# Stansfash/nonstationary-precip

Hardware: AMD Instinct MI355X
Metric: dsvi_elbo_steps_per_sec (higher is better)
Workload: dtype f32; 1 GPU; 2-layer DSVI DeepGP (hidden 3->2 + last 2->1), M=1024, S=10, minibatch 4096 (global, split over the GPUs) of synthetic N=1e5 spatio-temporal grid; fwd+ELBO+bwd+Adam; M=1024, S=10, per_gpu_batch=4096, global_batch=4096, N=100000, parallelism=dp1, kzz_cholesky_dtype=f64, hipgraph=True

## Files before the change

nonstationary-precip_amd/csrc/gemm.hip:

```cpp
#include <cstdlib>
#include <type_traits>
#include "common.h"

namespace {

constexpr int F64_BK = 16;
constexpr int F64_DEPTH = 2;
constexpr int F64ACC_BN = 64;
constexpr int F64ACC_BK = 16;

#ifdef NSGP_GEMM_STAMPS
__device__ unsigned long long* nsgp_stamp_buf = nullptr;
__device__ unsigned long long nsgp_stamp_cap = 0;
#define NSGP_STAMP(i) do { if (threadIdx.x == 0) stamp_v[i] = __builtin_amdgcn_s_memtime(); } while (0)
#define NSGP_STAMP_FLUSH() do { \
        if (threadIdx.x == 0 && nsgp_stamp_buf) { \
            const unsigned long long si = (unsigned long long)blockIdx.y * gridDim.x + blockIdx.x; \
            if (si < nsgp_stamp_cap) { \
                unsigned long long* sp = nsgp_stamp_buf + si * 16; \
                sp[0] = stamp_v[0]; sp[1] = stamp_v[1]; sp[2] = stamp_v[2]; sp[3] = __builtin_amdgcn_s_memtime(); \
                sp[4] = stamp_rt0; sp[5] = __builtin_amdgcn_s_memrealtime(); \
                sp[6] = ((unsigned long long)(unsigned)bm << 40) | ((unsigned long long)(unsigned)bn << 16) | (unsigned)nt; \
                sp[8] = stamp_bar; \
                sp[7] = ((unsigned long long)__builtin_amdgcn_s_getreg(63508) << 32) | (unsigned)__builtin_amdgcn_s_getreg(63492); \
            } \
        } } while (0)
#define NSGP_LOOP_BARRIER() do { \
        const unsigned long long b0_ = __builtin_amdgcn_s_memtime(); \
        __syncthreads(); \
        stamp_bar += __builtin_amdgcn_s_memtime() - b0_; \
    } while (0)
#else
#define NSGP_STAMP(i) do { } while (0)
#define NSGP_STAMP_FLUSH() do { } while (0)
#define NSGP_LOOP_BARRIER() __syncthreads()
#endif

template <typename T> struct Mfma;
template <> struct Mfma<float> {
    static constexpr int MT = 32, KS = 2, NREG = 16, PAD = 4;
    typedef float acc_t __attribute__((ext_vector_type(16)));
    static __device__ __forceinline__ acc_t mma(float a, float b, acc_t c) {
        return __builtin_amdgcn_mfma_f32_32x32x2f32(a, b, c, 0, 0, 0);
    }
    static __device__ __forceinline__ int krow(int lane) { return lane >> 5; }
    static __device__ __forceinline__ int mcol(int lane) { return lane & 31; }
    static __device__ __forceinline__ int crow(int r, int lane) { return (r & 3) + 8 * (r >> 2) + 4 * (lane >> 5); }
    static __device__ __forceinline__ int crow_lane(int lane) { return 4 * (lane >> 5); }
    static __device__ __forceinline__ constexpr int crow_reg(int r) { return (r & 3) + 8 * (r >> 2); }
    static __device__ __forceinline__ int ccol(int lane) { return lane & 31; }
};
template <> struct Mfma<double> {
    static constexpr int MT = 16, KS = 4, NREG = 4, PAD = 16;
    typedef double acc_t __attribute__((ext_vector_type(4)));
    static __device__ __forceinline__ acc_t mma(double a, double b, acc_t c) {
        return __builtin_amdgcn_mfma_f64_16x16x4f64(a, b, c, 0, 0, 0);
    }
    static __device__ __forceinline__ int krow(int lane) { return lane >> 4; }
    static __device__ __forceinline__ int mcol(int lane) { return lane & 15; }
    static __device__ __forceinline__ int crow(int r, int lane) { return (lane >> 4) + 4 * r; }
    static __device__ __forceinline__ int crow_lane(int lane) { return lane >> 4; }
    static __device__ __forceinline__ constexpr int crow_reg(int r) { return 4 * r; }
    static __device__ __forceinline__ int ccol(int lane) { return lane & 15; }
};

struct GemmArgs {
    int64_t M, N, K;
    int64_t sam, sak, sa1, sa2;
    int64_t sbk, sbn, sb1, sb2;
    int64_t ldc, sc1, sc2;
    int64_t nb2;
    int64_t tiles_m, tiles_n;
    int64_t ksplit, kper;
    int64_t slab;
    int flags;
    int nbk;
    int part_rows;
    int xcd_chunk;
    int xcd_group;
    int batch_perm;
    int vecA, vecB;
    int modeA, modeB;
};

struct Epi {
    int kind;
    const void *rv, *cs, *gc, *mat, *ks;
    void *p0, *p1;
    int modeA, modeB;
    int part_rows;
    int p64;
    const float *kz, *kx, *kls, *kos;
    int kD;
    int64_t kx_sx;
};
constexpr int KGEN_DMAX = 4;

template <typename T> struct Frag4 { T v[4]; };

template <typename T> __device__ __forceinline__ Frag4<T> ldg4(const T* p) {
    Frag4<T> f;
    if constexpr (sizeof(T) == 4) {
        const float4 q = *reinterpret_cast<const float4*>(p);
        f.v[0] = q.x; f.v[1] = q.y; f.v[2] = q.z; f.v[3] = q.w;
    } else {
        const double2 q0 = *reinterpret_cast<const double2*>(p);
        const double2 q1 = *reinterpret_cast<const double2*>(p + 2);
        f.v[0] = q0.x; f.v[1] = q0.y; f.v[2] = q1.x; f.v[3] = q1.y;
    }
    return f;
}

template <typename T, int MODE, int BR, int BK, int P>
struct TileLoader {
    static constexpr int TPK = BK / 4, TPR = BR / 4;
    static constexpr int RS = MODE == 0 ? 256 / TPK : 0;
    static constexpr int KS = MODE == 0 ? 0 : 256 / TPR;
    int r0, k0;
    const T* cur;
    int64_t pstep, kstep;
    __device__ __forceinline__ void init(int tid, const T* base, int64_t row0, int64_t sr, int64_t sk, int64_t kbeg) {
        if (MODE == 0) { r0 = tid / TPK; k0 = (tid % TPK) * 4; }
        else { r0 = (tid % TPR) * 4; k0 = tid / TPR; }
        kstep = sk;
        pstep = MODE == 0 ? RS * sr : KS * sk;
        cur = base + (row0 + r0) * sr + (kbeg + k0) * sk;
    }
    __device__ __forceinline__ int prow(int p) const { return r0 + p * RS; }
    __device__ __forceinline__ int pk(int p) const { return k0 + p * KS; }
    __device__ __forceinline__ void load_fast(Frag4<T>* f, int64_t koff) const {
#pragma unroll
        for (int p = 0; p < P; ++p) f[p] = ldg4(cur + p * pstep + koff * kstep);
    }
    __device__ __forceinline__ void load_edge(Frag4<T>* f, const T* base, int64_t row0, int64_t sr, int64_t sk, int64_t k0g,
                                              int rrem, int krem) const {
#pragma unroll
        for (int p = 0; p < P; ++p)
#pragma unroll
            for (int e = 0; e < 4; ++e) {
                const int r = prow(p) + (MODE == 0 ? 0 : e), k = pk(p) + (MODE == 0 ? e : 0);
                f[p].v[e] = (r < rrem && k < krem) ? base[(row0 + r) * sr + (k0g + k) * sk] : T(0);
            }
    }
    __device__ __forceinline__ void mask_piece(Frag4<T>& f, int p, int d, bool zgt, bool zlt) const {
#pragma unroll
        for (int e = 0; e < 4; ++e) {
            const int r = prow(p) + (MODE == 0 ? 0 : e), k = pk(p) + (MODE == 0 ? e : 0) + d;
            const bool z = (zgt && k > r) || (zlt && k < r);
            f.v[e] = z ? T(0) : f.v[e];
        }
    }
};

template <typename T, int BM, int BN, int BK, int MODE_A, int MODE_B>
struct TileLds {
    static constexpr int PADA = (MODE_A == 0 && sizeof(T) == 4) ? 1 : Mfma<T>::PAD;
    static constexpr int PADB = (MODE_B == 0 && sizeof(T) == 4) ? 1 : Mfma<T>::PAD;
    static constexpr int LDA = BM + PADA, LDB = BN + PADB;
    static constexpr size_t BYTES = 2 * BK * (LDA + LDB) * sizeof(T);
};

constexpr int resident_wg_per_cu(size_t elem_size, bool big, bool narrow) { return big ? (narrow ? 3 : 2) : (elem_size == 4 ? 6 : 3); }
constexpr int launch_min_wg(size_t elem_size, int bm, int bn) { return (elem_size == 4 && bm == 128 && bn == 64) ? 3 : 2; }

template <typename T, int BM, int BN, int BK, int MODE_A, int MODE_B, int EPI = 0, int KSC = 0, int EDGE = 1, int MIX = 0>
__global__ __launch_bounds__(256, launch_min_wg(sizeof(T), BM, BN)) void gemm_kernel(GemmArgs g, T alpha, const T* __restrict__ A,
                                                   const T* __restrict__ B, T beta, T* __restrict__ C,
                                                   T* __restrict__ slabs, Epi ep) {
    static_assert(MIX == 0 || (sizeof(T) == 8 && EPI == 1 && KSC == 0), "MIX: float64 colstats projection only");
    static_assert(MIX != 2 || (EDGE == 0 && MODE_B == 1), "MIX = 2 (generated Kzx operand): whole tiles, n-contiguous pieces");
    using TB = std::conditional_t<MIX == 1 || MIX == 2, float, T>;
    using TC = std::conditional_t<MIX != 0, float, T>;
    using MF = Mfma<T>;
    using LDS = TileLds<T, BM, BN, BK, MODE_A, MODE_B>;
    constexpr int MT = MF::MT, KS = MF::KS, NKK = BK / KS;
    constexpr int WM = BM / 2, WN = BN / 2;
    constexpr int TM = WM / MT, TN = WN / MT;
    constexpr int LDA = LDS::LDA, LDB = LDS::LDB;
    constexpr int PA = BM * BK / 1024, PB = BN * BK / 1024;
    extern __shared__ __attribute__((aligned(32))) unsigned char gemm_smem[];
    T (*As)[BK * LDA] = reinterpret_cast<T (*)[BK * LDA]>(gemm_smem);
    T (*Bs)[BK * LDB] = reinterpret_cast<T (*)[BK * LDB]>(gemm_smem + 2 * BK * LDA * sizeof(T));

    const int tid = threadIdx.x, lane = tid & 63, wave = __builtin_amdgcn_readfirstlane(tid >> 6);
    const int wm0 = (wave >> 1) * WM, wn0 = (wave & 1) * WN;
#ifdef NSGP_GEMM_STAMPS
    unsigned long long stamp_v[4] = {0, 0, 0, 0};
    unsigned long long stamp_bar = 0;
    const unsigned long long stamp_rt0 = __builtin_amdgcn_s_memrealtime();
    NSGP_STAMP(0);
#endif
    const int tiles_m = (int)g.tiles_m, tiles_n = (int)g.tiles_n;
    int tid_lin = (int)blockIdx.x, zz = (int)blockIdx.y;
    if (g.batch_perm == 3) {
        const int ntile = (int)gridDim.x;
        const int blk = tid_lin >> 8;
        if (blk & 1) {
            const int base = blk << 8;
            const int top = base + 255 < ntile - 1 ? base + 255 : ntile - 1;
            tid_lin = base + (top - tid_lin);
        }
    } else if (g.batch_perm) {
        const int ntile = (int)gridDim.x;
        int t = tid_lin + ((zz >> 1) & 1) * (ntile >> 1);
        if (t >= ntile) t -= ntile;
        tid_lin = (zz & 1) ? ntile - 1 - t : t;
        if (g.batch_perm == 2) {
            const int lin = zz * ntile + (int)blockIdx.x;
            tid_lin = lin / g.nbk;
            zz = lin % g.nbk;
        }
    }
    if (g.xcd_chunk > 0) {
        const int L = zz * (int)gridDim.x + tid_lin;
        const int logical = (L & 7) * g.xcd_chunk + (L >> 3);
        const int ntile = (int)gridDim.x;
        tid_lin = logical % ntile;
        zz = logical / ntile;
        if (zz >= g.nbk) return;
    }
    int bm, bn;
    if (g.flags & NSGP_GEMM_C_LOWER) {
        const int TT = tiles_m < tiles_n ? tiles_m : tiles_n;
        const int tri = TT * (TT + 1) / 2;
        if (g.flags & (NSGP_GEMM_A_LOWER | NSGP_GEMM_B_UPPER)) tid_lin = (int)gridDim.x - 1 - tid_lin;
        if (tid_lin < tri) {
            int r = (int)((sqrtf(8.0f * (float)tid_lin + 1.0f) - 1.0f) * 0.5f);
            while (r * (r + 1) / 2 > tid_lin) --r;
            while ((r + 1) * (r + 2) / 2 <= tid_lin) ++r;
            bm = r; bn = tid_lin - r * (r + 1) / 2;
        } else {
            const int q = tid_lin - tri;
            bm = TT + q / tiles_n; bn = q % tiles_n;
        }
    } else if (g.xcd_group > 0) {
        const int R = g.xcd_group;
        const int x = tid_lin & 7, j = tid_lin >> 3;
        const int panels8 = (tiles_n + 7) >> 3;
        const int per_group = panels8 * R;
        const int grp = j / per_group, jj = j - grp * per_group;
        bn = 8 * (jj / R) + x;
        bm = grp * R + (jj % R);
        if (bn >= tiles_n) return;
    } else {
        const int brow = tid_lin / tiles_n;
        bm = brow; bn = (tid_lin % tiles_n + tiles_n - brow % tiles_n) % tiles_n;
    }
    if (!(g.flags & NSGP_GEMM_C_LOWER)) {
        if (g.flags & NSGP_GEMM_A_LOWER) bm = tiles_m - 1 - bm;
        if (g.flags & NSGP_GEMM_B_UPPER) bn = tiles_n - 1 - bn;
    }
    const int ksp = (int)g.ksplit, nb2i = (int)g.nb2;
    const int64_t slice = zz % ksp, bb = zz / ksp;
    const int64_t b1 = (int)bb / nb2i, b2 = (int)bb % nb2i;
    const int64_t m0 = (int64_t)bm * BM, n0 = (int64_t)bn * BN;

    const T* Ab = A + b1 * g.sa1 + b2 * g.sa2;
    const TB* Bb = reinterpret_cast<const TB*>(B) + b1 * g.sb1 + b2 * g.sb2;
    TC* Cb = reinterpret_cast<TC*>(C) + b1 * g.sc1 + b2 * g.sc2;

    const bool aL = g.flags & NSGP_GEMM_A_LOWER, aU = g.flags & NSGP_GEMM_A_UPPER;
    const bool bL = g.flags & NSGP_GEMM_B_LOWER, bU = g.flags & NSGP_GEMM_B_UPPER;
    const bool cL = g.flags & NSGP_GEMM_C_LOWER;

    int64_t kbeg = slice * g.kper, kend = kbeg + g.kper < g.K ? kbeg + g.kper : g.K;
    if (aL) { const int64_t e = m0 + BM; if (e < kend) kend = e; }
    if (aU) { const int64_t s = m0 / BK * BK; if (s > kbeg) kbeg = s; }
    if (bL) { const int64_t s = n0 / BK * BK; if (s > kbeg) kbeg = s; }
    if (bU) { const int64_t e = n0 + BN; if (e < kend) kend = e; }
    const bool skip_block = cL && (n0 > m0 + BM - 1);
    if (skip_block) kend = kbeg;
    const int nt = kend > kbeg ? (int)((kend - kbeg + BK - 1) / BK) : 0;

    typename MF::acc_t acc[TM][TN];
#pragma unroll
    for (int i = 0; i < TM; ++i)
#pragma unroll
        for (int j = 0; j < TN; ++j)
#pragma unroll
            for (int r = 0; r < MF::NREG; ++r) acc[i][j][r] = T(0);

    TileLoader<T, MODE_A, BM, BK, PA> la;
    TileLoader<TB, MODE_B, BN, BK, PB> lb;
    la.init(tid, Ab, m0, g.sam, g.sak, kbeg);
    lb.init(tid, Bb, n0, g.sbn, g.sbk, kbeg);
    [[maybe_unused]] float kgxs[4][KGEN_DMAX], kgls[KGEN_DMAX], kgos = 0.f;
    [[maybe_unused]] const float* kgz = nullptr;
    [[maybe_unused]] int kgD = 0;
    if constexpr (MIX == 2) {
        kgD = ep.kD;
        kgz = ep.kz + bb * g.K * kgD;
        kgos = ep.kos[bb];
#pragma unroll
        for (int d = 0; d < KGEN_DMAX; ++d) kgls[d] = d < kgD ? ep.kls[bb * kgD + d] : 1.f;
        const float* xb = ep.kx + bb * ep.kx_sx;
#pragma unroll
        for (int e = 0; e < 4; ++e)
#pragma unroll
            for (int d = 0; d < KGEN_DMAX; ++d)
                kgxs[e][d] = d < kgD ? xb[(n0 + lb.prow(0) + e) * kgD + d] / kgls[d] : 0.f;
    }
    const int mrem = (int)(g.M - m0 < BM ? g.M - m0 : BM), nrem = (int)(g.N - n0 < BN ? g.N - n0 : BN);

    Frag4<T> ra0[PA];
    Frag4<TB> rb0[PB];
    Frag4<T> rks[KSC ? PB : 1];
    const T* ksb = KSC ? reinterpret_cast<const T*>(ep.ks) + bb * g.K : nullptr;
    const bool ks_vec = KSC && ((uintptr_t)ksb % (4 * sizeof(T)) == 0);

    constexpr int DEEP = (sizeof(T) == 8 && KSC == 0 && EDGE == 0 && (MIX != 0 || EPI == 0)) ? F64_DEPTH : 0;
    constexpr int NSET = DEEP > 2 ? DEEP : 2;
    bool st_adiag[NSET] = {}, st_bdiag[NSET] = {};
    int st_ad[NSET] = {}, st_bd[NSET] = {};
    auto load_ks = [&](int64_t k0) __attribute__((always_inline)) {
        if (MODE_B == 0) {
            const int64_t k = k0 + lb.k0;
            if (ks_vec && k + 3 < kend) {
                rks[0] = ldg4(ksb + k);
            } else {
#pragma unroll
                for (int e = 0; e < 4; ++e) rks[0].v[e] = k + e < kend ? ksb[k + e] : T(0);
            }
        } else {
#pragma unroll
            for (int p = 0; p < PB; ++p) {
                const int64_t k = k0 + lb.pk(p);
                rks[p].v[0] = k < kend ? ksb[k] : T(0);
            }
        }
    };
    auto gload = [&](int t, Frag4<T>* ra, Frag4<TB>* rb, int set = 0) __attribute__((always_inline)) {
        const int64_t k0 = kbeg + (int64_t)t * BK;
        if constexpr (EDGE == 0) {
            la.load_fast(ra, (int64_t)t * BK);
            lb.load_fast(rb, (int64_t)t * BK);
        } else {
            const int64_t left = kend - k0;
            const int krem = (int)(left < BK ? left : BK);
            la.load_edge(ra, Ab, m0, g.sam, g.sak, k0, mrem, krem);
            lb.load_edge(rb, Bb, n0, g.sbn, g.sbk, k0, nrem, krem);
        }
        st_adiag[set] = (aL || aU) && (k0 < m0 + BM) && (k0 + BK > m0);
        st_bdiag[set] = (bL || bU) && (k0 < n0 + BN) && (k0 + BK > n0);
        st_ad[set] = (int)(k0 - m0);
        st_bd[set] = (int)(k0 - n0);
        if constexpr (KSC != 0) load_ks(k0);
    };
    [[maybe_unused]] float kzs[PB][KGEN_DMAX];
    [[maybe_unused]] Frag4<TB> kval[PB];
    auto kgen_half = [&](Frag4<TB>* rb, int half) __attribute__((always_inline)) {
        if constexpr (MIX == 2) {
#pragma unroll
            for (int p = 0; p < PB; ++p) {
                if (half == 0) {
#pragma unroll
                    for (int d = 0; d < KGEN_DMAX; ++d) kzs[p][d] = d < kgD ? rb[p].v[d] / kgls[d] : 0.f;
                }
#pragma unroll
                for (int e = 2 * half; e < 2 * half + 2; ++e) {
                    float ex = 0.f;
#pragma unroll
                    for (int d = 0; d < KGEN_DMAX; ++d) {
                        const float df = kzs[p][d] - kgxs[e][d];
                        ex = __builtin_fmaf(df, df, ex);
                    }
                    kval[p].v[e] = kgos * t_fexp(-0.5f * ex);
                }
                if (half == 1) rb[p] = kval[p];
            }
        }
    };
    constexpr int NPIECE = PA + PB;
    auto store_piece = [&](int buf, int q, Frag4<T>* ra, Frag4<TB>* rb, auto masked_c, int set = 0) __attribute__((always_inline)) {
        constexpr bool MASKED = decltype(masked_c)::value;
        if (q < PA) {
            const int p = q;
            if constexpr (MASKED) {
                if (st_adiag[set]) la.mask_piece(ra[p], p, st_ad[set], aL, aU);
            }
            T* dst = &As[buf][la.pk(p) * LDA + la.prow(p)];
#pragma unroll
            for (int e = 0; e < 4; ++e) dst[MODE_A == 0 ? e * LDA : e] = ra[p].v[e];
        } else {
            const int p = q - PA;
            if constexpr (MASKED) {
                if (st_bdiag[set]) lb.mask_piece(rb[p], p, st_bd[set], bU, bL);
            }
            if constexpr (KSC != 0) {
#pragma unroll
                for (int e = 0; e < 4; ++e) rb[p].v[e] *= (TB)(MODE_B == 0 ? rks[0].v[e] : rks[p].v[0]);
            }
            T* dst = &Bs[buf][lb.pk(p) * LDB + lb.prow(p)];
#pragma unroll
            for (int e = 0; e < 4; ++e) dst[MODE_B == 0 ? e * LDB : e] = (T)rb[p].v[e];
        }
    };
    auto sstore = [&](int buf, Frag4<T>* ra, Frag4<TB>* rb, int set = 0) __attribute__((always_inline)) {
#pragma unroll
        for (int q = 0; q < NPIECE; ++q) store_piece(buf, q, ra, rb, std::true_type{}, set);
    };

    const int kr = MF::krow(lane), mc = MF::mcol(lane);
    constexpr int KS0 = NKK / 2;
    constexpr int PPS = (NPIECE + (NKK - KS0) - 1) / (NKK - KS0);
    constexpr int FULLMASK = (1 << (TM * TN)) - 1;
    auto ktile = [&](int buf, bool stage, auto tmask_c, auto masked_c, Frag4<T>* ra, Frag4<TB>* rb, int set = 0) __attribute__((always_inline)) {
        constexpr int tmask = decltype(tmask_c)::value;
        const T* as = &As[buf][kr * LDA + wm0 + mc];
        const T* bs = &Bs[buf][kr * LDB + wn0 + mc];
        T af[2][TM], bf[2][TN];
#pragma unroll
        for (int i = 0; i < TM; ++i) af[0][i] = as[i * MT];
#pragma unroll
        for (int j = 0; j < TN; ++j) bf[0][j] = bs[j * MT];
#pragma unroll
        for (int ks = 0; ks < NKK; ++ks) {
            const int cur = ks & 1, nxt = cur ^ 1;
            if (ks + 1 < NKK) {
#pragma unroll
                for (int i = 0; i < TM; ++i) af[nxt][i] = as[(ks + 1) * KS * LDA + i * MT];
#pragma unroll
                for (int j = 0; j < TN; ++j) bf[nxt][j] = bs[(ks + 1) * KS * LDB + j * MT];
            }
            if constexpr (MIX == 2) {
                static_assert(MIX != 2 || KS0 >= 2, "generated operand: two k-steps ahead of the staging stores");
                if (ks < 2 && stage) kgen_half(rb, ks);
            }
            if (ks >= KS0 && stage) {
#pragma unroll
                for (int q = (ks - KS0) * PPS; q < (ks - KS0 + 1) * PPS && q < NPIECE; ++q) store_piece(buf ^ 1, q, ra, rb, masked_c, set);
            }
            __builtin_amdgcn_sched_barrier(0);
#pragma unroll
            for (int i = 0; i < TM; ++i)
#pragma unroll
                for (int j = 0; j < TN; ++j)
                    if constexpr ((tmask >> 0) != 0) {
                        if ((tmask >> (i * TN + j)) & 1) acc[i][j] = MF::mma(af[cur][i], bf[cur][j], acc[i][j]);
                    }
            __builtin_amdgcn_sched_barrier(0);
        }
    };
    int cmask_tile = FULLMASK;
    if (cL) {
        cmask_tile = 0;
#pragma unroll
        for (int i = 0; i < TM; ++i)
#pragma unroll
            for (int j = 0; j < TN; ++j)
                if (n0 + wn0 + j * MT <= m0 + wm0 + (i + 1) * MT - 1) cmask_tile |= 1 << (i * TN + j);
    }
    auto tile_mask = [&](int64_t k0) __attribute__((always_inline)) {
        int mk = cmask_tile;
        if (aL || aU) {
#pragma unroll
            for (int i = 0; i < TM; ++i) {
                const int64_t r0 = m0 + wm0 + i * MT;
                const bool on = aL ? (k0 < r0 + MT) : (k0 + BK > r0);
                if (!on) mk &= ~(((1 << TN) - 1) << (i * TN));
            }
        }
        if (bL || bU) {
#pragma unroll
            for (int j = 0; j < TN; ++j) {
                const int64_t c0 = n0 + wn0 + j * MT;
                const bool on = bU ? (k0 < c0 + MT) : (k0 + BK > c0);
                if (!on) {
#pragma unroll
                    for (int i = 0; i < TM; ++i) mk &= ~(1 << (i * TN + j));
                }
            }
        }
        return mk;
    };
    if constexpr (DEEP > 0) {
        static_assert(DEEP % 2 == 0, "the LDS buffer index is static only for an even depth");
        if (nt > 0) {
            Frag4<T> rsa[DEEP][PA];
            Frag4<TB> rsb[DEEP][PB];
            auto issue = [&](int t, int set) __attribute__((always_inline)) {
                la.load_fast(rsa[set], (int64_t)t * BK);
                if constexpr (MIX == 2) {
#pragma unroll
                    for (int p = 0; p < PB; ++p) {
                        const int64_t k = kbeg + (int64_t)t * BK + lb.pk(p);
#pragma unroll
                        for (int d = 0; d < KGEN_DMAX; ++d) rsb[set][p].v[d] = d < kgD ? kgz[k * kgD + d] : 0.f;
                    }
                } else {
                    lb.load_fast(rsb[set], (int64_t)t * BK);
                }
                const int64_t k0 = kbeg + (int64_t)t * BK;
                st_adiag[set] = (aL || aU) && (k0 < m0 + BM) && (k0 + BK > m0);
                st_bdiag[set] = (bL || bU) && (k0 < n0 + BN) && (k0 + BK > n0);
                st_ad[set] = (int)(k0 - m0);
                st_bd[set] = (int)(k0 - n0);
            };
            issue(0, 0);
#pragma unroll
            for (int d = 1; d < DEEP; ++d)
                if (d < nt) issue(d, d);
            kgen_half(rsb[0], 0);
            kgen_half(rsb[0], 1);
            sstore(0, rsa[0], rsb[0], 0);
            __syncthreads();
            NSGP_STAMP(1);
            for (int tb = 0; tb < nt; tb += DEEP) {
#pragma unroll
                for (int j = 0; j < DEEP; ++j) {
                    const int t = tb + j;
                    if (t >= nt) break;
                    if (t + DEEP < nt) issue(t + DEEP, j);
                    ktile(j & 1, t + 1 < nt, std::integral_constant<int, FULLMASK>{}, std::true_type{}, rsa[(j + 1) % DEEP],
                          rsb[(j + 1) % DEEP], (j + 1) % DEEP);
                    NSGP_LOOP_BARRIER();
                }
            }
        }
    } else {
        if (nt > 0) {
            constexpr bool ROLL = sizeof(T) == 4 && KSC == 0;
            auto regular = [&](int t) __attribute__((always_inline)) {
                const int64_t k0 = kbeg + (int64_t)t * BK;
                if (k0 + BK > kend) return false;
                if constexpr (!ROLL) {
                    if ((aL || aU) && (k0 < m0 + BM) && (k0 + BK > m0)) return false;
                    if ((bL || bU) && (k0 < n0 + BN) && (k0 + BK > n0)) return false;
                }
                return true;
            };
            int r0 = 0, r1 = 0;
            const bool interior = EDGE == 0 || (!(MODE_A == 0 && MODE_B == 0) && g.vecA && g.vecB && m0 + BM <= g.M &&
                                                n0 + BN <= g.N);
            if (interior) {
                while (r0 < nt && !regular(r0)) ++r0;
                r1 = r0;
                while (r1 < nt && regular(r1)) ++r1;
            }
            const int h0 = r0, h1 = r1 - 1 > r0 ? r1 - 1 : r0;
            auto generic_tiles = [&](int tb, int te) __attribute__((always_inline)) {
                for (int t = tb; t < te; ++t) {
                    const int buf = t & 1;
                    const bool more = t + 1 < nt;
                    if (more) gload(t + 1, ra0, rb0);
                    const int mk = __builtin_amdgcn_readfirstlane(tile_mask(kbeg + (int64_t)t * BK));
                    if (mk == 0) ktile(buf, more, std::integral_constant<int, 0>{}, std::true_type{}, ra0, rb0);
                    else ktile(buf, more, std::integral_constant<int, FULLMASK>{}, std::true_type{}, ra0, rb0);
                    NSGP_LOOP_BARRIER();
                }
            };
            gload(0, ra0, rb0);
            sstore(0, ra0, rb0);
            __syncthreads();
            NSGP_STAMP(1);
            generic_tiles(0, h0);
            constexpr bool DEPTH2 = sizeof(T) == 8 && KSC == 0;
            int hend = h0;
            if constexpr (ROLL) {
                if (h1 > h0) {
                    int lo = h0, hi = h1;
                    {
                        const int64_t R0 = m0 + wm0, C0 = n0 + wn0;
                        if (aL) { const int64_t e = (R0 + WM - kbeg + BK - 1) / BK; if (e < hi) hi = (int)(e > 0 ? e : 0); }
                        if (aU) { const int64_t b = R0 > kbeg ? (R0 - kbeg) / BK : 0; if (b > lo) lo = (int)b; }
                        if (bU) { const int64_t e = (C0 + WN - kbeg + BK - 1) / BK; if (e < hi) hi = (int)(e > 0 ? e : 0); }
                        if (bL) { const int64_t b = C0 > kbeg ? (C0 - kbeg) / BK : 0; if (b > lo) lo = (int)b; }
                        if (cmask_tile == 0) { lo = h0; hi = h0; }
                        if (lo > h1) lo = h1;
                        if (hi < lo) hi = lo;
                        lo = __builtin_amdgcn_readfirstlane(lo);
                        hi = __builtin_amdgcn_readfirstlane(hi);
                    }
                    const T* pa = la.cur + (int64_t)(h0 + 1) * BK * la.kstep;
                    const TB* pb = lb.cur + (int64_t)(h0 + 1) * BK * lb.kstep;
                    const int64_t da = (int64_t)BK * la.kstep, db = (int64_t)BK * lb.kstep;
                    auto hot_seg = [&](int tb, int te, auto tmask_c, auto masked_c) __attribute__((always_inline)) {
                        for (int t = tb; t < te; ++t) {
#pragma unroll
                            for (int p = 0; p < PA; ++p) ra0[p] = ldg4(pa + p * la.pstep);
#pragma unroll
                            for (int p = 0; p < PB; ++p) rb0[p] = ldg4(pb + p * lb.pstep);
                            pa += da; pb += db;
                            if constexpr (decltype(masked_c)::value) {
                                const int64_t k0 = kbeg + (int64_t)(t + 1) * BK;
                                st_adiag[0] = (aL || aU) && (k0 < m0 + BM) && (k0 + BK > m0);
                                st_bdiag[0] = (bL || bU) && (k0 < n0 + BN) && (k0 + BK > n0);
                                st_ad[0] = (int)(k0 - m0);
                                st_bd[0] = (int)(k0 - n0);
                            }
                            ktile(t & 1, true, tmask_c, masked_c, ra0, rb0);
                            NSGP_LOOP_BARRIER();
                        }
                    };
                    int p0 = h0, p1 = h1;
                    {
                        auto first_k = [&](int t) { return kbeg + (int64_t)(t + 1) * BK; };
                        int64_t dlo = INT64_MAX, dhi = INT64_MIN;
                        if (aL || aU) { dlo = m0; dhi = m0 + BM; }
                        if (bL || bU) { if (n0 < dlo) dlo = n0; if (n0 + BN > dhi) dhi = n0 + BN; }
                        if (dhi > dlo) {
                            int below = h0, above = h1;
                            while (below < h1 && first_k(below) + BK <= dlo) ++below;
                            while (above > h0 && first_k(above - 1) >= dhi) --above;
                            if (below - h0 >= h1 - above) { p0 = h0; p1 = below; } else { p0 = above; p1 = h1; }
                        }
                        p0 = __builtin_amdgcn_readfirstlane(p0);
                        p1 = __builtin_amdgcn_readfirstlane(p1);
                    }
                    int cut[6] = {h0, p0, p1, lo, hi, h1};
#pragma unroll
                    for (int a = 1; a < 6; ++a)
#pragma unroll
                        for (int b = a; b > 0; --b)
                            if (cut[b] < cut[b - 1]) { const int tmp = cut[b]; cut[b] = cut[b - 1]; cut[b - 1] = tmp; }
#pragma unroll 1
                    for (int a = 0; a < 5; ++a) {
                        const int tb = cut[a], te = cut[a + 1];
                        if (tb >= te) continue;
                        const bool active = tb >= lo && te <= hi, plain = tb >= p0 && te <= p1;
                        if (active && plain) hot_seg(tb, te, std::integral_constant<int, FULLMASK>{}, std::false_type{});
                        else if (active) hot_seg(tb, te, std::integral_constant<int, FULLMASK>{}, std::true_type{});
                        else if (plain) hot_seg(tb, te, std::integral_constant<int, 0>{}, std::false_type{});
                        else hot_seg(tb, te, std::integral_constant<int, 0>{}, std::true_type{});
                    }
                    hend = h1;
                }
            }
            if (!ROLL && !DEPTH2 && h1 > h0) {
                const T* pa = la.cur + (int64_t)(h0 + 1) * BK * la.kstep;
                const TB* pb = lb.cur + (int64_t)(h0 + 1) * BK * lb.kstep;
                const int64_t da = (int64_t)BK * la.kstep, db = (int64_t)BK * lb.kstep;
                for (int t = h0; t < h1; ++t) {
#pragma unroll
                    for (int p = 0; p < PA; ++p) ra0[p] = ldg4(pa + p * la.pstep);
#pragma unroll
                    for (int p = 0; p < PB; ++p) rb0[p] = ldg4(pb + p * lb.pstep);
                    if constexpr (KSC != 0) load_ks(kbeg + (int64_t)(t + 1) * BK);
                    pa += da; pb += db;
                    ktile(t & 1, true, std::integral_constant<int, FULLMASK>{}, std::false_type{}, ra0, rb0);
                    NSGP_LOOP_BARRIER();
                }
                hend = h1;
            }
            if constexpr (DEPTH2) {
                const int h2 = h1 - 1;
                if (h2 - h0 >= 2) {
                    Frag4<T> rax[PA];
                    Frag4<TB> rbx[PB];
                    const T* pa = la.cur + (int64_t)(h0 + 1) * BK * la.kstep;
                    const TB* pb = lb.cur + (int64_t)(h0 + 1) * BK * lb.kstep;
                    const int64_t da = (int64_t)BK * la.kstep, db = (int64_t)BK * lb.kstep;
#pragma unroll
                    for (int p = 0; p < PA; ++p) ra0[p] = ldg4(pa + p * la.pstep);
#pragma unroll
                    for (int p = 0; p < PB; ++p) rb0[p] = ldg4(pb + p * lb.pstep);
                    pa += da; pb += db;
                    const int npairs = (h2 - h0) / 2;
                    int t = h0;
                    for (int q = 0; q < npairs; ++q, t += 2) {
#pragma unroll
                        for (int p = 0; p < PA; ++p) rax[p] = ldg4(pa + p * la.pstep);
#pragma unroll
                        for (int p = 0; p < PB; ++p) rbx[p] = ldg4(pb + p * lb.pstep);
                        pa += da; pb += db;
                        ktile(t & 1, true, std::integral_constant<int, FULLMASK>{}, std::false_type{}, ra0, rb0);
                        NSGP_LOOP_BARRIER();
#pragma unroll
                        for (int p = 0; p < PA; ++p) ra0[p] = ldg4(pa + p * la.pstep);
#pragma unroll
                        for (int p = 0; p < PB; ++p) rb0[p] = ldg4(pb + p * lb.pstep);
                        pa += da; pb += db;
                        ktile((t + 1) & 1, true, std::integral_constant<int, FULLMASK>{}, std::false_type{}, rax, rbx);
                        NSGP_LOOP_BARRIER();
                    }
                    hend = t;
                }
            }
            generic_tiles(hend, nt);
        }
    }

    NSGP_STAMP(2);
    if constexpr (EPI == 1) {
        const TC* rv = ep.rv ? reinterpret_cast<const TC*>(ep.rv) + bb * g.M : nullptr;
        T sdot[TN], ssq[TN];
#pragma unroll
        for (int j = 0; j < TN; ++j) { sdot[j] = T(0); ssq[j] = T(0); }
#pragma unroll
        for (int i = 0; i < TM; ++i)
#pragma unroll
            for (int r = 0; r < MF::NREG; ++r) {
                const int64_t row = m0 + wm0 + i * MT + MF::crow(r, lane);
                const T rvv = (rv && row < g.M) ? (T)rv[row] : T(0);
#pragma unroll
                for (int j = 0; j < TN; ++j) {
                    const int64_t col = n0 + wn0 + j * MT + MF::ccol(lane);
                    const T v = alpha * acc[i][j][r];
                    if (row < g.M && col < g.N) Cb[row * g.ldc + col] = (TC)v;
                    sdot[j] += v * rvv;
                    ssq[j] += v * v;
                }
            }
#pragma unroll
        for (int j = 0; j < TN; ++j) {
#pragma unroll
            for (int off = MT; off < 64; off <<= 1) {
                sdot[j] += __shfl_xor(sdot[j], off);
                ssq[j] += __shfl_xor(ssq[j], off);
            }
        }
        T* red = reinterpret_cast<T*>(gemm_smem);
        __syncthreads();
        if (lane < MT) {
#pragma unroll
            for (int j = 0; j < TN; ++j) {
                const int c = wn0 + j * MT + lane;
                red[(0 + (wave >> 1)) * BN + c] = sdot[j];
                red[(2 + (wave >> 1)) * BN + c] = ssq[j];
            }
        }
        __syncthreads();
        if (tid < BN && n0 + tid < g.N) {
            const int64_t o = (bb * (g.part_rows > 0 ? g.part_rows : g.tiles_m) + bm) * g.N + n0 + tid;
            if constexpr (MIX != 0) {
                if (ep.p64) {
                    if (ep.p0) reinterpret_cast<double*>(ep.p0)[o] = red[tid] + red[BN + tid];
                    reinterpret_cast<double*>(ep.p1)[o] = red[2 * BN + tid] + red[3 * BN + tid];
                    NSGP_STAMP_FLUSH();
                    return;
                }
            }
            if (ep.p0) reinterpret_cast<TC*>(ep.p0)[o] = (TC)(red[tid] + red[BN + tid]);
            reinterpret_cast<TC*>(ep.p1)[o] = (TC)(red[2 * BN + tid] + red[3 * BN + tid]);
        }
        NSGP_STAMP_FLUSH();
        return;
    } else if constexpr (EPI == 2) {
        const T* mat = reinterpret_cast<const T*>(ep.mat) + b1 * g.sc1 + b2 * g.sc2;
        const T* rv = reinterpret_cast<const T*>(ep.rv) + bb * g.M;
        const T* gc = reinterpret_cast<const T*>(ep.gc) + bb * g.N;
        const T* cs = reinterpret_cast<const T*>(ep.cs) + bb * g.N;
        const bool inside = (m0 + BM <= g.M) && (n0 + BN <= g.N);
#pragma unroll
        for (int j = 0; j < TN; ++j) {
            const int64_t col = n0 + wn0 + j * MT + MF::ccol(lane);
            const int64_t colc = col < g.N ? col : g.N - 1;
            const T gcol = gc[colc], c2 = T(2) * cs[colc];
#pragma unroll
            for (int i = 0; i < TM; ++i) {
                T av[MF::NREG], rvv[MF::NREG];
                if (inside) {
#pragma unroll
                    for (int r = 0; r < MF::NREG; ++r) {
                        const int64_t row = m0 + wm0 + i * MT + MF::crow(r, lane);
                        av[r] = mat[row * g.ldc + col];
                        rvv[r] = rv[row];
                    }
#pragma unroll
                    for (int r = 0; r < MF::NREG; ++r) {
                        const int64_t row = m0 + wm0 + i * MT + MF::crow(r, lane);
                        Cb[row * g.ldc + col] = (alpha * acc[i][j][r] - av[r]) * c2 + rvv[r] * gcol;
                    }
                } else {
#pragma unroll
                    for (int r = 0; r < MF::NREG; ++r) {
                        const int64_t row = m0 + wm0 + i * MT + MF::crow(r, lane);
                        if (row < g.M && col < g.N)
                            Cb[row * g.ldc + col] = (alpha * acc[i][j][r] - mat[row * g.ldc + col]) * c2 + rv[row] * gcol;
                    }
                }
            }
        }
        NSGP_STAMP_FLUSH();
        return;
    }
    if constexpr (MIX == 0) {
    const bool to_slab = g.ksplit > 1;
    T* out = to_slab ? slabs + slice * g.slab + bb * g.M * g.N : Cb;
    const int64_t ldo = to_slab ? g.N : g.ldc;
    const bool plain_tile = (m0 + BM <= g.M) && (n0 + BN <= g.N) &&
                            (to_slab || (!cL && beta == T(0) && !(g.flags & NSGP_GEMM_C_HALFDIAG)));
    if (plain_tile) {
        const T sc = to_slab ? T(1) : alpha;
        T* o0 = out + (m0 + wm0 + MF::crow_lane(lane)) * ldo + n0 + wn0 + MF::ccol(lane);
#pragma unroll
        for (int i = 0; i < TM; ++i)
#pragma unroll
            for (int j = 0; j < TN; ++j)
#pragma unroll
                for (int r = 0; r < MF::NREG; ++r)
                    o0[(int64_t)(i * MT + MF::crow_reg(r)) * ldo + j * MT] = sc * acc[i][j][r];
        NSGP_STAMP_FLUSH();
        return;
    }
#pragma unroll
    for (int i = 0; i < TM; ++i)
#pragma unroll
        for (int j = 0; j < TN; ++j)
#pragma unroll
            for (int r = 0; r < MF::NREG; ++r) {
                const int64_t row = m0 + wm0 + i * MT + MF::crow(r, lane);
                const int64_t col = n0 + wn0 + j * MT + MF::ccol(lane);
                if (row < g.M && col < g.N) {
                    T v = acc[i][j][r];
                    if (to_slab) {
                        out[row * ldo + col] = v;
                    } else {
                        if (cL && col > row) {
                            if (beta == T(0)) out[row * ldo + col] = T(0);
                        } else {
                            v *= alpha;
                            if ((g.flags & NSGP_GEMM_C_HALFDIAG) && row == col) v *= T(0.5);
                            if (beta != T(0)) v += beta * out[row * ldo + col];
                            out[row * ldo + col] = v;
                        }
                    }
                }
            }
    }
    NSGP_STAMP_FLUSH();
}

struct Out64 { double* p; int64_t ld, s1, s2; };

template <typename T>
__global__ void splitk_reduce_kernel(GemmArgs g, T alpha, const T* __restrict__ slabs, T beta, T* __restrict__ C,
                                     int64_t nb, Out64 o) {
    const int64_t idx = (int64_t)blockIdx.x * blockDim.x + threadIdx.x;
    const int64_t per = g.M * g.N;
    if (idx >= nb * per) return;
    const int64_t bb = idx / per, e = idx % per;
    const int64_t row = e / g.N, col = e % g.N;
    const int64_t b1 = bb / g.nb2, b2 = bb % g.nb2;
    T* c = C + b1 * g.sc1 + b2 * g.sc2 + row * g.ldc + col;
    double* c64 = o.p ? o.p + b1 * o.s1 + b2 * o.s2 + row * o.ld + col : nullptr;
    if ((g.flags & NSGP_GEMM_C_LOWER) && col > row) {
        if (beta == T(0)) {
            *c = T(0);
            if (c64) *c64 = 0.0;
        }
        return;
    }
    T s = T(0);
    for (int64_t k = 0; k < g.ksplit; ++k) s += slabs[k * g.slab + idx];
    s *= alpha;
    if ((g.flags & NSGP_GEMM_C_HALFDIAG) && row == col) s *= T(0.5);
    if (beta != T(0)) s += beta * *c;
    *c = s;
    if (c64) *c64 = (double)s;
}

struct ReduceVec {
    unsigned M, N, n4, nb2;
    unsigned groups;
    unsigned fill;
    int ksplit, flags;
    int64_t slab, ldc, sc1, sc2;
};
constexpr int REDUCE_UNROLL = 8;

static_assert(REDUCE_UNROLL == 8, "splitk_reduce_vec_kernel spells out the remainders 1..7");

template <int CNT, typename V, typename T>
__device__ __forceinline__ void reduce_add(V& s, const T* p, int64_t slab) {
    V v[CNT];
#pragma unroll
    for (int i = 0; i < CNT; ++i) v[i] = *reinterpret_cast<const V*>(p + i * slab);
#pragma unroll
    for (int i = 0; i < CNT; ++i) s += v[i];
}

template <typename T>
__global__ __launch_bounds__(256) void splitk_reduce_vec_kernel(ReduceVec r, T alpha, const T* __restrict__ slabs, T beta,
                                                                T* __restrict__ C, Out64 o) {
    typedef T V __attribute__((ext_vector_type(4)));
    typedef double D2 __attribute__((ext_vector_type(2)));
    const unsigned t = blockIdx.x * 256u + threadIdx.x;
    const unsigned bb = blockIdx.y;
    const unsigned b1 = bb / r.nb2, b2 = bb - b1 * r.nb2;
    const bool cL = (r.flags & NSGP_GEMM_C_LOWER) != 0;
    unsigned row, cg;
    bool fill = false;
    if (t < r.groups) {
        if (!cL) {
            row = t / r.n4; cg = t - row * r.n4;
        } else {
            const unsigned w = r.n4 + 1, fr = t / w, j = t - fr * w, q = fr >> 2;
            if (j <= q) { row = fr; cg = j; } else { row = r.M - 1 - fr; cg = j - (q + 1); }
        }
    } else {
        const unsigned u = t - r.groups;
        if (u >= r.fill) return;
        const unsigned w = r.n4 - 1, fr = u / w, j = u - fr * w, q = fr >> 2, nup = w - q;
        if (j < nup) { row = fr; cg = q + 1 + j; } else { row = r.M - 1 - fr; cg = ((r.M - 1 - fr) >> 2) + 1 + (j - nup); }
        fill = true;
    }
    const unsigned col0 = 4 * cg;
    T* c = C + ((int64_t)b1 * r.sc1 + (int64_t)b2 * r.sc2 + (int64_t)row * r.ldc + col0);
    double* c64 = o.p ? o.p + ((int64_t)b1 * o.s1 + (int64_t)b2 * o.s2 + (int64_t)row * o.ld + col0) : nullptr;
    if (fill) {
        *reinterpret_cast<V*>(c) = V(T(0));
        if (c64) {
            reinterpret_cast<D2*>(c64)[0] = D2(0.0);
            reinterpret_cast<D2*>(c64)[1] = D2(0.0);
        }
        return;
    }
    const T* p = slabs + ((bb * r.M + row) * r.N + col0);
    const bool half = (r.flags & NSGP_GEMM_C_HALFDIAG) != 0;
    if (cL && col0 + 3 > row) {
        for (unsigned i = 0; i < 4; ++i) {
            const unsigned col = col0 + i;
            if (col > row) {
                if (beta == T(0)) {
                    c[i] = T(0);
                    if (c64) c64[i] = 0.0;
                }
                continue;
            }
            T s = T(0);
            for (int k = 0; k < r.ksplit; ++k) s += p[k * r.slab + i];
            s *= alpha;
            if (half && row == col) s *= T(0.5);
            if (beta != T(0)) s += beta * c[i];
            c[i] = s;
            if (c64) c64[i] = (double)s;
        }
        return;
    }
    V s = V(T(0));
    int k = 0;
    for (; k + REDUCE_UNROLL <= r.ksplit; k += REDUCE_UNROLL, p += REDUCE_UNROLL * r.slab)
        reduce_add<REDUCE_UNROLL, V>(s, p, r.slab);
    switch (r.ksplit - k) {
        case 1: reduce_add<1, V>(s, p, r.slab); break;
        case 2: reduce_add<2, V>(s, p, r.slab); break;
        case 3: reduce_add<3, V>(s, p, r.slab); break;
        case 4: reduce_add<4, V>(s, p, r.slab); break;
        case 5: reduce_add<5, V>(s, p, r.slab); break;
        case 6: reduce_add<6, V>(s, p, r.slab); break;
        case 7: reduce_add<7, V>(s, p, r.slab); break;
        default: break;
    }
    s *= alpha;
    if (half && (row >> 2) == cg) {
        const unsigned d = row & 3;
        s.x = d == 0 ? s.x * T(0.5) : s.x; s.y = d == 1 ? s.y * T(0.5) : s.y;
        s.z = d == 2 ? s.z * T(0.5) : s.z; s.w = d == 3 ? s.w * T(0.5) : s.w;
    }
    if (beta != T(0)) s += beta * *reinterpret_cast<const V*>(c);
    *reinterpret_cast<V*>(c) = s;
    if (c64) {
        reinterpret_cast<D2*>(c64)[0] = D2{(double)s.x, (double)s.y};
        reinterpret_cast<D2*>(c64)[1] = D2{(double)s.z, (double)s.w};
    }
}

struct Plan { int big, narrow; int64_t ksplit, kper; };

struct GemmEnv {
    bool no_xcd;
    int xcd_group;
    char batch_perm;
    bool force_narrow;
    size_t lds_extra;
};
static inline GemmEnv gemm_env() {
    const char* no_xcd = getenv("NSGP_GEMM_NO_XCD");
    const char* grp = getenv("NSGP_GEMM_XCD_GROUP");
    const char* bpe = getenv("NSGP_GEMM_BATCH_PERM");
    const char* fn = getenv("NSGP_GEMM_FORCE_NARROW");
    const char* xe = getenv("NSGP_GEMM_LDS_EXTRA");
    return GemmEnv{no_xcd && no_xcd[0] == '1', grp ? atoi(grp) : 0, bpe ? bpe[0] : (char)0, fn && fn[0] == '1',
                   xe ? (size_t)atoi(xe) : 0};
}

template <typename T> constexpr int tile_bk(int bm, bool plain) { return bm == 128 ? 32 : ((sizeof(T) == 8 && plain) ? F64_BK : 16); }

static inline int64_t active_tiles(int64_t M, int64_t N, int64_t bm, int flags) {
    const int64_t tm = cdiv64(M, bm), tn = cdiv64(N, bm);
    if (!(flags & NSGP_GEMM_C_LOWER)) return tm * tn;
// ... 524 lines not shown
```

Measured before the change: 241.2 steps/s.

## Specialize GEMM k-tiles on finer per-fragment compile-time masks for triangular operands

Adds a compile-time set of partial fragment masks (single rows, columns, all-but-one) and dispatches k-tile segments to specializations that skip MFMA work for fragments entirely outside the triangular region. It also splits the hot loop at per-fragment diagonal crossings and peels the last k-tile so its mask is handled separately. The aim is to cut wasted MFMA on structurally zero triangular blocks (Cholesky/triangular products), at the cost of more template instantiations, code size and register pressure.

Result: no change. 242.8 steps/s (median of 6 runs) (+0.7%).

```diff
diff --git a/nonstationary-precip_amd/csrc/gemm.hip b/nonstationary-precip_amd/csrc/gemm.hip
--- a/nonstationary-precip_amd/csrc/gemm.hip
+++ b/nonstationary-precip_amd/csrc/gemm.hip
@@ -1,6 +1,7 @@
 #include <cstdlib>
 #include <type_traits>
 #include "common.h"
+#include "gemm_masks.h"
 
 namespace {
 
@@ -163,6 +164,22 @@
 constexpr int resident_wg_per_cu(size_t elem_size, bool big, bool narrow) { return big ? (narrow ? 3 : 2) : (elem_size == 4 ? 6 : 3); }
 constexpr int launch_min_wg(size_t elem_size, int bm, int bn) { return (elem_size == 4 && bm == 128 && bn == 64) ? 3 : 2; }
 
+template <int TM, int TN, int KINDS, int Q = 0, typename F>
+__device__ __forceinline__ void with_mask(int mk, F&& f) {
+    constexpr int m = nsgp_masks::member(TM, TN, Q), all = nsgp_masks::full(TM, TN);
+    static_assert(m >= 0, "the set ends with the full mask");
+    constexpr bool ab01 = TM == 2 && TN == 2 && m == nsgp_masks::all_but_01(TN);
+    constexpr bool admitted = m == 0 || m == all || KINDS == 2 || (KINDS == 1 && ab01) || (KINDS == 3 && !ab01);
+    if constexpr (m == all) {
+        f(std::integral_constant<int, all>{});
+    } else {
+        if constexpr (admitted) {
+            if ((mk & ~m) == 0) { f(std::integral_constant<int, m>{}); return; }
+        }
+        with_mask<TM, TN, KINDS, Q + 1>(mk, f);
+    }
+}
+
 template <typename T, int BM, int BN, int BK, int MODE_A, int MODE_B, int EPI = 0, int KSC = 0, int EDGE = 1, int MIX = 0>
 __global__ __launch_bounds__(256, launch_min_wg(sizeof(T), BM, BN)) void gemm_kernel(GemmArgs g, T alpha, const T* __restrict__ A,
                                                    const T* __restrict__ B, T beta, T* __restrict__ C,
@@ -544,8 +561,9 @@
                     const bool more = t + 1 < nt;
                     if (more) gload(t + 1, ra0, rb0);
                     const int mk = __builtin_amdgcn_readfirstlane(tile_mask(kbeg + (int64_t)t * BK));
-                    if (mk == 0) ktile(buf, more, std::integral_constant<int, 0>{}, std::true_type{}, ra0, rb0);
-                    else ktile(buf, more, std::integral_constant<int, FULLMASK>{}, std::true_type{}, ra0, rb0);
+                    with_mask<TM, TN, 0>(mk, [&](auto tmask_c) __attribute__((always_inline)) {
+                        ktile(buf, more, tmask_c, std::true_type{}, ra0, rb0);
+                    });
                     NSGP_LOOP_BARRIER();
                 }
             };
@@ -553,9 +571,10 @@
             sstore(0, ra0, rb0);
             __syncthreads();
             NSGP_STAMP(1);
-            generic_tiles(0, h0);
+            const int last = nt - 1;
+            generic_tiles(0, h0 < last ? h0 : last);
             constexpr bool DEPTH2 = sizeof(T) == 8 && KSC == 0;
-            int hend = h0;
+            int hend = h0 < last ? h0 : last;
             if constexpr (ROLL) {
                 if (h1 > h0) {
                     int lo = h0, hi = h1;
@@ -571,6 +590,19 @@
                         lo = __builtin_amdgcn_readfirstlane(lo);
                         hi = __builtin_amdgcn_readfirstlane(hi);
                     }
+                    int rcut = lo, ccut = lo;
+                    if constexpr (TM == 2) {
+                        const int64_t R1 = m0 + wm0 + MT - kbeg;
+                        if (aL) rcut = (int)((R1 + BK - 1) / BK);
+                        if (aU) rcut = (int)(R1 > 0 ? R1 / BK : 0);
+                    }
+                    if constexpr (TN == 2) {
+                        const int64_t C1 = n0 + wn0 + MT - kbeg;
+                        if (bU) ccut = (int)((C1 + BK - 1) / BK);
+                        if (bL) ccut = (int)(C1 > 0 ? C1 / BK : 0);
+                    }
+                    rcut = __builtin_amdgcn_readfirstlane(rcut < lo ? lo : rcut > hi ? hi : rcut);
+                    ccut = __builtin_amdgcn_readfirstlane(ccut < lo ? lo : ccut > hi ? hi : ccut);
                     const T* pa = la.cur + (int64_t)(h0 + 1) * BK * la.kstep;
                     const TB* pb = lb.cur + (int64_t)(h0 + 1) * BK * lb.kstep;
                     const int64_t da = (int64_t)BK * la.kstep, db = (int64_t)BK * lb.kstep;
@@ -607,21 +639,34 @@
                         p0 = __builtin_amdgcn_readfirstlane(p0);
                         p1 = __builtin_amdgcn_readfirstlane(p1);
                     }
-                    int cut[6] = {h0, p0, p1, lo, hi, h1};
-#pragma unroll
-                    for (int a = 1; a < 6; ++a)
-#pragma unroll
-                        for (int b = a; b > 0; --b)
-                            if (cut[b] < cut[b - 1]) { const int tmp = cut[b]; cut[b] = cut[b - 1]; cut[b - 1] = tmp; }
+                    int tb = h0;
 #pragma unroll 1
-                    for (int a = 0; a < 5; ++a) {
-                        const int tb = cut[a], te = cut[a + 1];
-                        if (tb >= te) continue;
+                    while (tb < h1) {
+                        int te = h1;
+                        if (p0 > tb && p0 < te) te = p0;
+                        if (p1 > tb && p1 < te) te = p1;
+                        if (lo > tb && lo < te) te = lo;
+                        if constexpr (TM == 2) { if (rcut > tb && rcut < te) te = rcut; }
+                        if constexpr (TN == 2) { if (ccut > tb && ccut < te) te = ccut; }
+                        if (hi > tb && hi < te) te = hi;
                         const bool active = tb >= lo && te <= hi, plain = tb >= p0 && te <= p1;
-                        if (active && plain) hot_seg(tb, te, std::integral_constant<int, FULLMASK>{}, std::false_type{});
-                        else if (active) hot_seg(tb, te, std::integral_constant<int, FULLMASK>{}, std::true_type{});
-                        else if (plain) hot_seg(tb, te, std::integral_constant<int, 0>{}, std::false_type{});
-                        else hot_seg(tb, te, std::integral_constant<int, 0>{}, std::true_type{});
+                        int mk = active ? cmask_tile : 0;
+                        if constexpr (TM == 2) {
+                            if (aL && tb >= rcut) mk &= nsgp_masks::row(TN, 1);
+                            if (aU && tb < rcut) mk &= nsgp_masks::row(TN, 0);
+                        }
+                        if constexpr (TN == 2) {
+                            if (bU && tb >= ccut) mk &= nsgp_masks::col(TM, TN, 1);
+                            if (bL && tb < ccut) mk &= nsgp_masks::col(TM, TN, 0);
+                        }
+                        mk = __builtin_amdgcn_readfirstlane(mk);
+                        const int cov = nsgp_masks::cover(TM, TN, mk);
+                        const bool half = cov != 0 && cov != FULLMASK && !(TM == 2 && TN == 2 && cov == nsgp_masks::all_but_01(TN));
+                        if (plain && !half)
+                            with_mask<TM, TN, 1>(mk, [&](auto tmask_c) __attribute__((always_inline)) { hot_seg(tb, te, tmask_c, std::false_type{}); });
+                        else
+                            with_mask<TM, TN, 3>(mk, [&](auto tmask_c) __attribute__((always_inline)) { hot_seg(tb, te, tmask_c, std::true_type{}); });
+                        tb = te;
                     }
                     hend = h1;
                 }
@@ -630,16 +675,18 @@
                 const T* pa = la.cur + (int64_t)(h0 + 1) * BK * la.kstep;
                 const TB* pb = lb.cur + (int64_t)(h0 + 1) * BK * lb.kstep;
                 const int64_t da = (int64_t)BK * la.kstep, db = (int64_t)BK * lb.kstep;
-                for (int t = h0; t < h1; ++t) {
-#pragma unroll
-                    for (int p = 0; p < PA; ++p) ra0[p] = ldg4(pa + p * la.pstep);
-#pragma unroll
-                    for (int p = 0; p < PB; ++p) rb0[p] = ldg4(pb + p * lb.pstep);
-                    if constexpr (KSC != 0) load_ks(kbeg + (int64_t)(t + 1) * BK);
-                    pa += da; pb += db;
-                    ktile(t & 1, true, std::integral_constant<int, FULLMASK>{}, std::false_type{}, ra0, rb0);
-                    NSGP_LOOP_BARRIER();
-                }
+                with_mask<TM, TN, 1>(__builtin_amdgcn_readfirstlane(cmask_tile), [&](auto tmask_c) __attribute__((always_inline)) {
+                    for (int t = h0; t < h1; ++t) {
+#pragma unroll
+                        for (int p = 0; p < PA; ++p) ra0[p] = ldg4(pa + p * la.pstep);
+#pragma unroll
+                        for (int p = 0; p < PB; ++p) rb0[p] = ldg4(pb + p * lb.pstep);
+                        if constexpr (KSC != 0) load_ks(kbeg + (int64_t)(t + 1) * BK);
+                        pa += da; pb += db;
+                        ktile(t & 1, true, tmask_c, std::false_type{}, ra0, rb0);
+                        NSGP_LOOP_BARRIER();
+                    }
+                });
                 hend = h1;
             }
             if constexpr (DEPTH2) {
@@ -676,7 +723,14 @@
                     hend = t;
                 }
             }
-            generic_tiles(hend, nt);
+            generic_tiles(hend, last);
+            {
+                const int mk = __builtin_amdgcn_readfirstlane(tile_mask(kbeg + (int64_t)last * BK));
+                with_mask<TM, TN, 2>(mk, [&](auto tmask_c) __attribute__((always_inline)) {
+                    ktile(last & 1, false, tmask_c, std::true_type{}, ra0, rb0);
+                });
+                NSGP_LOOP_BARRIER();
+            }
         }
     }
 
diff --git a/nonstationary-precip_amd/csrc/gemm_masks.h b/nonstationary-precip_amd/csrc/gemm_masks.h
--- /dev/null
+++ b/nonstationary-precip_amd/csrc/gemm_masks.h
@@ -0,0 +1,33 @@
+#pragma once
+
+namespace nsgp_masks {
+
+constexpr int full(int tm, int tn) { return (1 << (tm * tn)) - 1; }
+constexpr int row(int tn, int i) { return ((1 << tn) - 1) << (i * tn); }
+constexpr int col(int tm, int tn, int j) {
+    int m = 0;
+    for (int i = 0; i < tm; ++i) m |= 1 << (i * tn + j);
+    return m;
+}
+constexpr int all_but_01(int tn) { return 15 & ~(1 << (0 * tn + 1)); }
+
+constexpr int MAX_MEMBERS = 7;
+constexpr int member(int tm, int tn, int q) {
+    int m[MAX_MEMBERS] = {0, -1, -1, -1, -1, -1, -1};
+    int n = 1;
+    if (tm == 2 && tn <= 2) { m[n++] = row(tn, 0); m[n++] = row(tn, 1); }
+    if (tn == 2 && tm <= 2) { m[n++] = col(tm, tn, 0); m[n++] = col(tm, tn, 1); }
+    if (tm == 2 && tn == 2) m[n++] = all_but_01(tn);
+    m[n++] = full(tm, tn);
+    return q < n ? m[q] : -1;
+}
+
+constexpr int cover(int tm, int tn, int mk) {
+    for (int q = 0; q < MAX_MEMBERS; ++q) {
+        const int m = member(tm, tn, q);
+        if (m >= 0 && (mk & ~m) == 0) return m;
+    }
+    return full(tm, tn);
+}
+
+}
```
